# ZGC-SP/mpcith_kyber_kosk

Measured on AMD Instinct MI355X. Metric: kyber768_kosk_proofs_per_sec_prove_plus_verify, higher is better.
Workload: dtype u16

## Files before the change

mpcith_kyber_kosk_amd/csrc/kosk_ctx.cpp:

```cpp
#include "kosk_ctx.hpp"

#include <atomic>

#include <chrono>
#include <cstdio>
#include <cstring>
#include <ctime>
#include <thread>

#include "kosk_math.hpp"

namespace kosk {

#define HIPCHK(x) KOSK_HIPCHK(x)

static double now_sec()
{
    return std::chrono::duration<double>(std::chrono::steady_clock::now().time_since_epoch()).count();
}

template <typename T>
static hipError_t dalloc(T **p, size_t n)
{
    return hipMalloc(reinterpret_cast<void **>(p), n * sizeof(T));
// ... 32 lines not shown
        if (pool) pool_destroy(pool);
        if (ev) (void)hipEventDestroy(ev);
        if (ev_kg) (void)hipEventDestroy(ev_kg);
        for (auto e : timer_ev)
            if (e) (void)hipEventDestroy(e);
        return;
    }
    void *dev[] = {t_expand.dfrag, t_recon_d.dfrag, t_recon_2d.dfrag, d_fresh_rows, d_gemm1_rows, d_gemm2_rows, d_off, d_fields, d_asm_groups, d_asm_elems,
                   d_rowtab, d_P, d_tape, d_seedbuf, d_dig1, d_dig2, d_proof, d_A, d_se, d_kg, d_sehat, d_t, d_alpha, d_I, d_pwT, d_coef, d_lin_rows,
                   d_gather, d_gather2, d_O, d_w, d_ell, d_sec, d_sec_u1, d_sec_u2, d_fail, d_inv, d_invlimb, d_vfields,
                   d_vrowtab, d_rows_bg, d_rows_isrc, d_rows_idst, d_rows_u, d_fact, d_invfact, d_node_of, d_isort, d_hrange, d_odig};
    for (void *p : dev)
        if (p) (void)hipFree(p);
    void *host[] = {h_err, h_tape, h_seedbuf, h_dig, h_dig2, h_proof, h_alpha, h_I, h_fail, h_Iimg, h_kg, h_odig};
    for (void *p : host)
        if (p) (void)hipHostFree(p);
    if (d_compact) (void)hipFree(d_compact);
    if (d_compact_bad) (void)hipFree(d_compact_bad);
    if (h_compact) (void)hipHostFree(h_compact);
    if (h_compact_bad) (void)hipHostFree(h_compact_bad);
    if (pool) pool_destroy(pool);
    if (ev) (void)hipEventDestroy(ev);
    if (ev_kg) (void)hipEventDestroy(ev_kg);
    for (auto e : timer_ev)
        if (e) (void)hipEventDestroy(e);
    if (stream) (void)hipStreamDestroy(stream);
}

static int upload_table(Ctx &c, GemmTable &t, const std::vector<uint16_t> &A, int M, int Kdim)
{
    t.M = M;
    t.Mpad = (M + 127) / 128 * 128;
    t.KS = (Kdim + 63) / 64;
    std::vector<uint8_t> pk;
    pack_frag_table(A, M, Kdim, t.Mpad, t.KS, pk);
    HIPCHK(dalloc(&t.dfrag, pk.size()));
    HIPCHK(hipMemcpyAsync(t.dfrag, pk.data(), pk.size(), hipMemcpyHostToDevice, c.stream));
    HIPCHK(hipStreamSynchronize(c.stream));
    return 0;
}

static hipError_t commit_hash_batch(Ctx &c, const HashArgs &ha, int n, int K, bool view, hipStream_t st)
{
    c.prof_begin(view ? PR_HASH_VIEW : PR_HASH_TCOMM, n);
    int variant = 0;
    const hipError_t e = launch_commit_hash(ha, n, K, view, st, &variant);
    if (!c.capturing) c.path_n[(variant & 1) ? PATH_HASH_DMA : PATH_HASH_PLAIN]++;
    c.prof_end(view ? PR_HASH_VIEW : PR_HASH_TCOMM);
    return e;
}

int device_error_check(Ctx &c)
{
    if (!c.h_err) return 0;
    const uint32_t e = *reinterpret_cast<volatile uint32_t *>(c.h_err);
    if (!e) return 0;
    *reinterpret_cast<volatile uint32_t *>(c.h_err) = 0;
    c.err = (e & DEVERR_XOF_BLOCKS) ? "gen_matrix: SHAKE128 block limit reached before 256 coefficients were accepted (indcpa.c:124-145 would squeeze on; "
                                      "probability < 2^-300 with the default limit of 32 blocks): no result was produced"
                                    : "a kernel reported an internal error";
    return -1;
}

hipError_t copy_round_table(Ctx &c, uint8_t *h_dst, const uint8_t *d_src, int n)
{
    return hipMemcpyAsync(h_dst, d_src, (size_t)n * NPARTY * 32, hipMemcpyDeviceToHost, c.stream);
}

// ... 39 lines not shown
        const double keep = est * 0.3 > 100.0 ? est * 0.3 : 100.0;
        double nap_us = est - keep;
        if (nap_us > 200000.0) nap_us = 200000.0;
        struct timespec ts;
        ts.tv_sec = 0;
        ts.tv_nsec = (long)(nap_us * 1e3);
        nanosleep(&ts, nullptr);
        const hipError_t q = hipEventQuery(ev);
        if (q == hipSuccess) overslept = true;
        else if (q != hipErrorNotReady) return q;
    }
    const hipError_t e = overslept ? hipSuccess : hipEventSynchronize(ev);
    const double took = (now_sec() - t0) * 1e6;
    if (overslept) {
        for (int i = 0; i < Ctx::WAIT_HIST; i++) h->us[i] = 0;
        h->at = 0;
    } else {
        h->us[h->at] = took > 1.0 ? took : 1.0;
        h->at = (h->at + 1) % Ctx::WAIT_HIST;
    }
    return e;
}
hipError_t stream_sync_site(Ctx &c, int site, int n)
{
    if (c.blocking_sync || !c.wait_nap) return stream_sync(c);
    const hipError_t e = hipEventRecord(c.ev_sync, c.stream);
    return e != hipSuccess ? e : wait_event(c, c.ev_sync, site, n);
}

int gemm_modq(Ctx &c, const GemmTable &t, const GemmSrc &s, const GemmDst &d, int npg, int ngroups)
{
    if (npg <= 0 || ngroups <= 0) return 0;
    GemmArgs ga{};
    ga.Afrag = t.dfrag; ga.Mpad = t.Mpad; ga.M = t.M; ga.KS = t.KS;
    ga.src = s.src; ga.src_gstride = s.gstride; ga.src_rows = s.rows; ga.src_rstride = s.rstride; ga.src_koff = s.koff;
    ga.src_canonical = s.canonical;
    ga.C = d.C; ga.c_gstride = d.gstride; ga.c_rows = d.rows; ga.c_rstride = d.rstride; ga.c_off = d.off;
    ga.npg = npg; ga.ngroups = ngroups;
    if (!table_gemm_ok(ga)) { c.err = "internal: table_gemm_ok() refuses the operands of a mod-q product"; return -1; }
    HIPCHK(launch_table_gemm(ga, c.stream));
    if (!c.capturing) c.path_n[PATH_TABLE_GEMM]++;
    return 0;
}

template <typename T>
static int upload_vec(Ctx &c, T **d, const std::vector<T> &v)
{
    HIPCHK(dalloc(d, v.size() ? v.size() : 1));
    if (!v.empty()) {
        HIPCHK(hipMemcpyAsync(*d, v.data(), v.size() * sizeof(T), hipMemcpyHostToDevice, c.stream));
        HIPCHK(hipStreamSynchronize(c.stream));
    }
    return 0;
}

static int build_tables(Ctx &c)
{
    const Params &P = c.P;
    const RowMap &rm = c.rm;
    const int K = P.K, M = P.M, E = P.E, Z = P.Z;

    {
        std::vector<uint16_t> A((size_t)EXP_M * XLEN, 0);
        for (int m = 0; m < EXP_M; m++) {
            const int x = EXP_OFF + m;
            if (x < XLEN) A[(size_t)m * XLEN + x] = 1;
            else if (x < NPTS) lagrange_row(&A[(size_t)m * XLEN], XLEN, 0, x);
// ... 790 lines not shown
```

mpcith_kyber_kosk_amd/csrc/kosk_ctx.hpp:

```cpp
#pragma once
#include <hip/hip_runtime.h>

#include <string>
#include <functional>
#include <vector>

#include "kosk_device.hpp"
#include "kosk_host.hpp"
#include "kosk_params.hpp"

#define KOSK_HIPCHK(x)                                                      \
    do {                                                                    \
        hipError_t e_ = (x);                                                \
        if (e_ != hipSuccess) {                                             \
            (void)hipGetLastError();                                        \
            c.err = std::string(#x) + ": " + hipGetErrorString(e_);         \
            return -1;                                                      \
        }                                                                   \
    } while (0)

namespace kosk {

typedef void (*randombytes_fn)(void *user, uint8_t *out, size_t len);
typedef void (*round_fn)(void *user, int role, int round, const void *d_digests, size_t bytes);
// ... 2 lines not shown
    const uint8_t *tapes;
    size_t tape_stride;
    uint8_t *pk, *sk;
    int count = 0;
    const KeygenIn *next = nullptr;
    round_fn hook = nullptr;
    void *hook_user = nullptr;
    const uint8_t *seeds = nullptr;
    size_t seed_stride = 0;
};
struct VerifySeg {
    int count;
    const uint8_t *pk;
    uint8_t *ok;
    const VerifySeg *next = nullptr;
    round_fn hook = nullptr;
    void *hook_user = nullptr;
};

enum Phase { PH_HOST_PRE = 0, PH_GPU_COMMIT, PH_FS_ALPHA, PH_GPU_RELATION, PH_FS_OPEN, PH_GPU_ASSEMBLE, PH_D2H,
             PH_P1_ISSUE, PH_P2_ISSUE, PH_P3_ISSUE, PH_V1_ISSUE, PH_V1_WAIT, PH_V_FS_ALPHA, PH_V2_ISSUE, PH_V2_WAIT, PH_V_FS_OPEN,
             PH_COUNT };

enum ProfId { PR_HASH_TCOMM = 0, PR_HASH_VIEW, PR_GEMM_EXPAND1, PR_GEMM_EXPAND2, PR_LINCOMB, PR_NTT_F, PR_ASSEMBLE,
              PR_V_HASH_TCOMM, PR_V_HASH_VIEW, PR_V_INTERP_BUILD, PR_V_GEMM_INTERP, PR_V_GEMM_EXPAND, PR_V_GEMM_RECON,
              PR_V_LINCOMB, PR_FS_ALPHA, PR_FS_OPENED, PR_V_FS_ALPHA, PR_V_FS_OPENED, PR_COUNT };

enum PathId { PATH_HASH_DMA = 0, PATH_HASH_PLAIN, PATH_TABLE_GEMM, PATH_LIMB_GEMM, PATH_COPY_DIRECT, PATH_COPY_STAGED,
              PATH_GRAPH_REPLAY, PATH_DIGEST_COPY, PATH_SMALL_COPY_KERNEL, PATH_FS_DEVICE, PATH_FS_HOST, PATH_TAPE_EXPAND, PATH_COUNT };

struct GemmTable {
    uint8_t *dfrag = nullptr;
    int M = 0, Mpad = 0, KS = 0;
};

struct GemmSrc {
    const uint16_t *src;
    size_t gstride;
    const int16_t *rows;
    int rstride, koff;
    int canonical = 1;
};
struct GemmDst {
    uint16_t *C;
    size_t gstride;
    const int16_t *rows;
    int rstride, off;
};

struct CompactField {
    uint32_t src_off, dst_off, n;
    int raw;
};
struct CompactPlan {
    CompactField f[NFIELDS];
    size_t bytes;
};
CompactPlan make_compact_plan(const Params &P);
int compact_encode(const Params &P, const uint8_t *img, uint8_t *out);
void compact_decode(const Params &P, const uint8_t *in, uint8_t *img);

struct Ctx {
    int device = 0;
    Params P{};
    RowMap rm{};
    int max_batch = 0;
// ... 234 lines not shown
```

mpcith_kyber_kosk_amd/csrc/kosk_device.hpp:

```cpp
#pragma once
#include <hip/hip_runtime.h>

#include "kosk_params.hpp"

namespace kosk {

struct XofGuard {
    uint32_t *err = nullptr;
    int max_blocks = 32;
};
enum : uint32_t { DEVERR_XOF_BLOCKS = 1u };


struct HashArgs {
    const uint16_t *rows;
    size_t group_stride;
    int row_stride;
    int col_off;
    int lanes_per_group;
    const uint8_t *prefix;
    uint8_t *out;
    int out_lanes_per_group;
};

struct NttArgs {
    const int16_t *in;
    const int32_t *src_off;
    size_t in_gstride;
    int16_t *out;
    const int32_t *dst_off;
    size_t out_gstride;
    int npg;
    int npoly;
    int out_canonical;
    uint32_t *cmp_fail;
    int cmp_delta, cmp_bit;
    uint32_t npg_magic;
};
inline uint32_t ntt_npg_magic(int npg) { return npg <= 1 ? 0xFFFFFFFFu : (uint32_t)((1ull << 32) / (uint32_t)npg); }

KOSK_HD inline int limb_swz(int r) { return (-(r >> 2)) & 3; }
KOSK_HD inline size_t limb_offset(int r, int k, int limb, int RT)
{
    const int ks = k >> 6, kc = (k >> 4) & 3, rr = r & 15;
    return ((size_t)(ks * RT + (r >> 4)) * 2 + limb) * 1024 + rr * 64 + ((kc ^ limb_swz(rr)) << 4) + (k & 15);
}
KOSK_HD inline void limb_split(int32_t centred, int &c0, int &c1)
{
    c0 = ((centred + 32) & 63) - 32;
    c1 = (centred - c0) >> 6;
}

struct GemmArgs {
    const uint8_t *Afrag;
    int Mpad, M, KS;
    const uint16_t *src;
    size_t src_gstride;
    const int16_t *src_rows;
    int src_rstride, src_koff;
    uint16_t *C;
    size_t c_gstride;
    const int16_t *c_rows;
    int c_rstride;
    int c_off;
    int npg;
    int src_canonical;
    int ngroups;
};

struct LincombArgs {
    uint16_t *P;
    size_t proof_stride;
    uint16_t *O;
    size_t o_stride;
    RowMap rm;
    int J;
    const int32_t *pwT;
    int ncols;
    const uint16_t *col_map;
    int col_map_stride;
    int nxb, njc, ngroups;
};

struct FieldDesc {
    uint32_t off;
    int sel;
    int width;
    int rowtab_off;
// ... 193 lines not shown
```

mpcith_kyber_kosk_amd/csrc/kosk_host.cpp:

```cpp
#include "kosk_host.hpp"

#include <linux/futex.h>
#include <sched.h>
#include <sys/random.h>
#include <sys/syscall.h>
#include <unistd.h>

#include <algorithm>
#include <atomic>
#include <chrono>
#include <mutex>
#include <stdexcept>
#include <cstdio>
#include <cstdlib>
#include <cstring>
#include <vector>
#include <thread>

#include "kosk_math.hpp"

namespace kosk {

namespace {

// ... 494 lines not shown
                e >>= 1;
            }
            inv[a] = (uint16_t)r;
        }
    }
};
const InvTable &inv_table()
{
    static const InvTable t;
    return t;
}
}

uint16_t gf_inv_host(uint16_t a) { return inv_table().inv[a % Q]; }

void lagrange_row(uint16_t *row, int n, int a, int t)
{
    std::vector<uint32_t> pre(n + 1), suf(n + 1), fact(n + 1);
    fact[0] = 1;
    for (int i = 1; i <= n; i++) fact[i] = fact[i - 1] * (uint32_t)i % Q;
    auto diff = [&](int m) { return (uint32_t)((((t - a - m) % Q) + Q) % Q); };
    pre[0] = 1;
    for (int m = 0; m < n; m++) pre[m + 1] = pre[m] * diff(m) % Q;
    suf[n] = 1;
    for (int m = n - 1; m >= 0; m--) suf[m] = suf[m + 1] * diff(m) % Q;
    for (int j = 0; j < n; j++) {
        const uint32_t num = pre[j] * suf[j + 1] % Q;
        uint32_t den = fact[j] * fact[n - 1 - j] % Q;
        if ((n - 1 - j) & 1) den = (Q - den) % Q;
        row[j] = (uint16_t)(num * gf_inv_host((uint16_t)den) % Q);
    }
}

void pack_frag_table(const std::vector<uint16_t> &A, int M, int Kdim, int Mpad, int KS, std::vector<uint8_t> &out)
{
    const int RT = Mpad / 16;
    out.assign((size_t)KS * RT * 2048, 0);
    for (int m = 0; m < M; m++)
        for (int k = 0; k < Kdim; k++) {
            const int32_t c = gf_center(A[(size_t)m * Kdim + k]);
            const int c0 = ((c + 32) & 63) - 32, c1 = (c - c0) >> 6;
            const int ks = k >> 6, kc = (k >> 4) & 3, rr = m & 15;
            const size_t base = ((size_t)(ks * RT + (m >> 4)) * 2) * 1024 + (size_t)(kc * 16 + rr) * 16 + (k & 15);
            out[base] = (uint8_t)(int8_t)c0;
            out[base + 1024] = (uint8_t)(int8_t)c1;
        }
}

class Pool {
public:
    static Pool &get() { static Pool p; return p; }
    Pool() = default;
    ~Pool()
    {
        stop_.store(true);
        gen_.fetch_add(1);
        wake(INT32_MAX);
        for (auto &t : th_) t.join();
    }
    void run(int n, int nthreads, const std::function<void(int)> &fn)
    {
        std::lock_guard<std::mutex> job_lock(job_mu_);
        grow(nthreads - 1);
        Job job{&fn, n, std::min<int>((int)th_.size(), nthreads - 1)};
        cur_.store(&job);
        gen_.fetch_add(1);
        if (sleepers_.load() > 0) wake(job.want);
        work(job);
        while (job.done.load(std::memory_order_acquire) < n) __builtin_ia32_pause();
        cur_.store(nullptr);
        while (inside_.load() != 0) __builtin_ia32_pause();
        if (job.failed.load()) throw std::runtime_error("exception in a host worker job");
    }

private:
// ... 135 lines not shown
```

mpcith_kyber_kosk_amd/csrc/kosk_host.hpp:

```cpp
#pragma once
#include <cstddef>
#include <cstdint>
#include <functional>
#include <vector>

#include "kosk_params.hpp"

namespace kosk {

void sha3_256(uint8_t out[32], const uint8_t *in, size_t inlen);
void sha3_512(uint8_t out[64], const uint8_t *in, size_t inlen);
void shake128(uint8_t *out, size_t outlen, const uint8_t *in, size_t inlen);
void shake256(uint8_t *out, size_t outlen, const uint8_t *in, size_t inlen);
void shake256_prf(uint8_t *out, size_t outlen, const uint8_t key[32], uint8_t nonce);

struct HostKey {
    int16_t A[MAXK * MAXK * 256];
    int16_t se[2 * MAXK * 256];
    int16_t t[MAXK * 256];
};
void host_keygen(const Params &P, const uint8_t seed64[64], uint8_t *pk, uint8_t *sk, HostKey &key);
void host_decode_pk(const Params &P, const uint8_t *pk, HostKey &key);

void fs_alpha(const Params &P, const uint8_t *tcomm_all , uint16_t *alpha );
void fs_opened(const uint8_t *digests_all , uint16_t I[NOPEN], uint16_t rest[NREST]);

void lagrange_row(uint16_t *row, int n, int a, int t);
uint16_t gf_inv_host(uint16_t a);

void pack_frag_table(const std::vector<uint16_t> &A, int M, int Kdim, int Mpad, int KS, std::vector<uint8_t> &out);

class Pool;
Pool *pool_create();
void pool_destroy(Pool *);
int pool_reserve(Pool *, int nthreads);
int host_cpu_count();
void parallel_for(Pool *pool, int n, int nthreads, const std::function<void(int)> &fn);
inline void parallel_for(int n, int nthreads, const std::function<void(int)> &fn) { parallel_for(nullptr, n, nthreads, fn); }

void sha3_256_multi(uint8_t *out, const uint8_t *const *in, size_t len, int count);
int sha3_multi_width();

void assemble_digest_table(uint8_t *table, const uint16_t *I, const uint8_t *unopened, const uint8_t *opened);

void fs_alpha_batch(const Params &P, int n, const uint8_t *digs, size_t dig_stride, uint16_t *alpha, size_t alpha_stride, int nthreads, Pool *pool = nullptr,
                    const std::function<void(int)> *prep = nullptr);
void fs_opened_batch(int n, const uint8_t *digs, size_t dig_stride, uint16_t *I, uint16_t *rest, size_t sel_stride, int nthreads, Pool *pool = nullptr,
                     bool windows = false, const std::function<void(int)> *prep = nullptr);

void os_randombytes(uint8_t *out, size_t len);

constexpr int SEED_BYTES = 32;
void tape_from_seed(const Params &P, const uint8_t seed[SEED_BYTES], uint8_t *tape);

}
```

mpcith_kyber_kosk_amd/csrc/kosk_kernels.hip:

```cpp
#include <hip/hip_runtime.h>

#include <cstdlib>
#include <utility>

#include "kosk_device.hpp"
#include "kosk_keccak_dev.hpp"
#include "kosk_keccak_split_dev.hpp"
#include "kosk_keygen_dev.hpp"
#include "kosk_keygen_wave_dev.hpp"
#include "kosk_math.hpp"
#include "kosk_limb_dev.hpp"

namespace kosk {

template <int PREFIX_WORDS, int NROWS, bool PIPE>
__global__ __launch_bounds__(64) void k_commit_hash(HashArgs a)
{
    const int lane = blockIdx.x * 64 + threadIdx.x;
    const int g = blockIdx.y;
    if (lane >= a.lanes_per_group) return;
    const uint16_t *__restrict__ base = a.rows + (size_t)g * a.group_stride + a.col_off + lane;
    const size_t dig = ((size_t)g * a.out_lanes_per_group + lane) * 32;

    constexpr int W = PREFIX_WORDS + NROWS;
// ... 675 lines not shown
__global__ __launch_bounds__(128) void k_matvec_ntt(const int16_t *__restrict__ A, size_t A_stride,
                                                    uint16_t *__restrict__ P, size_t proof_stride, int v_row0, int row0, int K)
{
    matvec_ntt_item(A, A_stride, P, proof_stride, v_row0, row0, K, threadIdx.x, blockIdx.x, blockIdx.y);
}

__global__ __launch_bounds__(256) void k_relation_ntt(NttArgs na, const int16_t *__restrict__ A, size_t A_stride, uint16_t *P,
                                                      size_t proof_stride, RowMap rm)
{
    __shared__ __attribute__((aligned(16))) int16_t lds[NTT_PPB * NTT_LSTRIDE];
    const int b = blockIdx.x, K = rm.K, tid = threadIdx.x;
    NttArgs a = na;
    a.in += (size_t)b * na.in_gstride;
    a.out += (size_t)b * na.out_gstride;
    a.npoly = a.npg;
    ntt256_tile(a, 0, lds);
    __syncthreads();
    for (int idx = tid; idx < K * 128; idx += 256) matvec_ntt_item(A, A_stride, P, proof_stride, rm.nttsr, rm.nttasr, K, idx & 127, idx >> 7, b);
    if (tid <= NOPEN) {
        uint16_t *Pb = P + (size_t)b * proof_stride + NSEC + tid;
        for (int i = 0; i < K; i++) {
            const uint16_t sv = Pb[(size_t)(rm.sr + i) * RS], ev = Pb[(size_t)(rm.er + i) * RS];
            Pb[(size_t)(rm.nttsr + i) * RS] = sv;
            Pb[(size_t)(rm.nttasr + i) * RS] = sv;
            Pb[(size_t)(rm.ntter + i) * RS] = ev;
        }
    }
}


constexpr int TG_WAVES = 8;

template <int KS, int TG_RT, int NBT>
__global__ __launch_bounds__(512, (KS <= 7 && NBT == 3) ? 2 : 1) void k_table_gemm(GemmArgs a, int nchunks, int chunks_per_block, int nblk, int msplit, int wide_stores)
{
    constexpr int TG_CHUNK = 16 * TG_RT, TG_NB = 16 * NBT;
    __shared__ __attribute__((aligned(16))) uint8_t ldsB[KS * NBT * 2048];
    const int tid = threadIdx.x, lane = tid & 63, w = tid >> 6;
    const int ntot = a.npg * a.ngroups;
    const int vid = xcd_virtual_id();
    const int bxr = vid / msplit, byr = vid - bxr * msplit;
    if (bxr >= nblk) return;
    const int n0 = bxr * TG_NB;

    constexpr int ITEMS = TG_NB * KS * 4, PER = (ITEMS + 511) / 512;
    uint4 x0[PER], x1[PER];
#pragma unroll
    for (int q = 0; q < PER; q++) {
        const int item = tid + q * 512;
        const int row_l = item / (KS * 4), kc16 = item - row_l * (KS * 4);
        const int n = n0 + row_l;
        x0[q] = make_uint4(0, 0, 0, 0);
        x1[q] = x0[q];
        if (item < ITEMS && n < ntot) {
            const int g = n / a.npg, i = n - g * a.npg;
            const uint16_t *src = a.src + (size_t)g * a.src_gstride + (size_t)(a.src_rows ? (int)a.src_rows[i] : i) * a.src_rstride + a.src_koff + kc16 * 16;
            x0[q] = *reinterpret_cast<const uint4 *>(src);
            x1[q] = *reinterpret_cast<const uint4 *>(src + 8);
        }
    }
#pragma unroll
    for (int q = 0; q < PER; q++) {
        const int item = tid + q * 512;
        if (item < ITEMS) {
            const int row_l = item / (KS * 4), kc16 = item - row_l * (KS * 4);
            uint4 lo, hi;
            gm_split16(x0[q], x1[q], lo, hi);
// ... 68 lines not shown
#pragma unroll
        for (int ks = 0; ks < KS; ks++) {
            v4i(&bc)[2 * NBT] = ks == 0 ? fb0 : fb[ks & 1];
            v4i(&bn)[2 * NBT] = ks + 1 == KS ? fb0 : fb[(ks & 1) ^ 1];
            load_b(ks + 1 < KS ? ks + 1 : 0, bn);
            __builtin_amdgcn_sched_barrier(0);
#pragma unroll
            for (int i = 0; i < TG_RT; i++) {
#pragma unroll
                for (int j = 0; j < NBT; j++) s0[i][j] = __builtin_amdgcn_mfma_i32_16x16x64_i8(fa[ks][2 * i], bc[2 * j], ks == 0 ? zero4 : s0[i][j], 0, 0, 0);
#pragma unroll
                for (int j = 0; j < NBT; j++) s1[i][j] = __builtin_amdgcn_mfma_i32_16x16x64_i8(fa[ks][2 * i], bc[2 * j + 1], ks == 0 ? zero4 : s1[i][j], 0, 0, 0);
#pragma unroll
                for (int j = 0; j < NBT; j++) s1[i][j] = __builtin_amdgcn_mfma_i32_16x16x64_i8(fa[ks][2 * i + 1], bc[2 * j], s1[i][j], 0, 0, 0);
#pragma unroll
                for (int j = 0; j < NBT; j++) s2[i][j] = __builtin_amdgcn_mfma_i32_16x16x64_i8(fa[ks][2 * i + 1], bc[2 * j + 1], ks == 0 ? zero4 : s2[i][j], 0, 0, 0);
            }
            load_chunk_ks(cn, ks, fa[ks]);
            __builtin_amdgcn_sched_barrier(0);
        }
        uint2 pk[NBT];
#pragma unroll
        for (int j = 0; j < NBT; j++) {
            uint32_t v[4];
#pragma unroll
            for (int r = 0; r < 4; r++) v[r] = gf_reduce_limbs(s0[0][j][r], s1[0][j][r], s2[0][j][r]);
            pk[j] = make_uint2(v[0] | (v[1] << 16), v[2] | (v[3] << 16));
            if (j & 1) store_pair(j - 1, c, pk[j - 1], pk[j]);
            else if (j == NBT - 1) store_one(j, c, pk[j]);
        }
    }
}

template <int KS, int NBT, bool CANON>
__global__ __launch_bounds__(512, 1) void k_table_gemm_p(GemmArgs a, int nchunks, int nblk, int wide_stores, uint32_t npg_magic)
{
    auto split = [&](int n, int &g, int &i) {
        uint32_t gg = __umulhi((uint32_t)n, npg_magic);
        int r = n - (int)gg * a.npg;
        if (r >= a.npg) { gg++; r -= a.npg; }
        g = (int)gg;
        i = r;
    };
    constexpr int TG_RT = 1, TG_CHUNK = 16, TG_NB = 16 * NBT, BUF = KS * NBT * 2048;
    __shared__ __attribute__((aligned(16))) uint8_t ldsB[2 * BUF];
    const int tid = threadIdx.x, lane = tid & 63, w = tid >> 6;
    const int ntot = a.npg * a.ngroups;
    const long total = (long)nblk * nchunks;
    const long u0 = (long)blockIdx.x * total / gridDim.x, u1 = (long)(blockIdx.x + 1) * total / gridDim.x;
    if (u0 >= u1) return;
    int rb = (int)(u0 / nchunks), ca = (int)(u0 - (long)rb * nchunks);
    long u = u0;

    constexpr int ITEMS = TG_NB * KS * 4, PER = (ITEMS + 511) / 512;
    auto item_src = [&](int blk, int item) -> const uint16_t * {
        const int row_l = item / (KS * 4), kc16 = item - row_l * (KS * 4);
        const int n = blk * TG_NB + row_l;
        if (item >= ITEMS || n >= ntot) return nullptr;
        int g, i;
        split(n, g, i);
        return a.src + (size_t)g * a.src_gstride + (size_t)(a.src_rows ? (int)a.src_rows[i] : i) * a.src_rstride + a.src_koff + kc16 * 16;
    };
    auto item_put = [&](int buf, int item, const uint4 &x0, const uint4 &x1) {
        if (item >= ITEMS) return;
        const int row_l = item / (KS * 4), kc16 = item - row_l * (KS * 4);
        uint4 lo, hi;
        if constexpr (CANON) gm_split16_pk(x0, x1, lo, hi);
        else gm_split16(x0, x1, lo, hi);
        uint8_t *d = ldsB + buf * BUF + ((kc16 >> 2) * NBT + (row_l >> 4)) * 2048 + (row_l & 15) * 64 + (((kc16 & 3) ^ limb_swz(row_l & 15)) << 4);
        *reinterpret_cast<uint4 *>(d) = lo;
        *reinterpret_cast<uint4 *>(d + 1024) = hi;
    };
    {
        uint4 x0[PER], x1[PER];
#pragma unroll
        for (int q = 0; q < PER; q++) {
            const uint16_t *src = item_src(rb, tid + q * 512);
            x0[q] = make_uint4(0, 0, 0, 0);
            x1[q] = x0[q];
            if (src) { x0[q] = *reinterpret_cast<const uint4 *>(src); x1[q] = *reinterpret_cast<const uint4 *>(src + 8); }
        }
#pragma unroll
        for (int q = 0; q < PER; q++) item_put(0, tid + q * 512, x0[q], x1[q]);
    }
    const int ART = a.Mpad / 16;
    const int frag = (lane & 15) * 64 + (((lane >> 4) ^ limb_swz(lane & 15)) << 4);
    v4i fa[KS][2 * TG_RT];
    auto load_chunk_ks = [&](int c, int ks, v4i (&dst)[2 * TG_RT]) {
        const uint8_t *src = a.Afrag + ((size_t)(ks * ART + TG_RT * c) * 2) * 1024 + lane * 16;
#pragma unroll
        for (int q = 0; q < 2 * TG_RT; q++) dst[q] = *reinterpret_cast<const v4i *>(src + q * 1024);
    };
    {
        const int c_first = ca + w < nchunks ? ca + w : 0;
#pragma unroll
        for (int ks = 0; ks < KS; ks++) load_chunk_ks(c_first, ks, fa[ks]);
    }
    __syncthreads();
    const v4i zero4 = {0, 0, 0, 0}, bias4 = {LIMB_BIAS, LIMB_BIAS, LIMB_BIAS, LIMB_BIAS};
    const int grp = lane >> 4;
    int buf = 0;
    while (u < u1) {
        const int cb = (long)(nchunks - ca) <= u1 - u ? nchunks : ca + (int)(u1 - u);
        const bool have_next = u + (cb - ca) < u1;
        const uint8_t *lds_cur = ldsB + buf * BUF;
        uint16_t *crow[NBT];
#pragma unroll
        for (int j = 0; j < NBT; j++) {
            const int n = rb * TG_NB + j * 16 + (lane & 15);
            crow[j] = nullptr;
            if (n < ntot) {
                int g, i;
                split(n, g, i);
                crow[j] = a.C + (size_t)g * a.c_gstride + (size_t)(a.c_rows ? (int)a.c_rows[i] : i) * a.c_rstride + a.c_off + (lane >> 4) * 4;
            }
        }
        auto store_pair = [&](int j, int c, uint2 pj, uint2 pk) {
            if (wide_stores) {
                const auto sx = __builtin_amdgcn_permlane16_swap(pj.x, pk.x, false, false);
                const auto sy = __builtin_amdgcn_permlane16_swap(pj.y, pk.y, false, false);
                uint16_t *p = (grp & 1) ? (crow[j + 1] ? crow[j + 1] - 4 : nullptr) : crow[j];
                if (p) *reinterpret_cast<uint4 *>(p + c * TG_CHUNK) = make_uint4(sx[0], sy[0], sx[1], sy[1]);
            } else {
                if (crow[j]) *reinterpret_cast<uint2 *>(crow[j] + c * TG_CHUNK) = pj;
                if (crow[j + 1]) *reinterpret_cast<uint2 *>(crow[j + 1] + c * TG_CHUNK) = pk;
            }
        };
        auto store_one = [&](int j, int c, uint2 pj) {
            if (crow[j]) *reinterpret_cast<uint2 *>(crow[j] + c * TG_CHUNK) = pj;
        };
        v4i fb[2][2 * NBT], fb0[2 * NBT];
        auto load_b = [&](int ks, v4i (&dst)[2 * NBT]) {
            const uint8_t *lb = lds_cur + ks * NBT * 2048 + frag;
#pragma unroll
            for (int j = 0; j < NBT; j++) {
                dst[2 * j] = *reinterpret_cast<const v4i *>(lb + j * 2048);
                dst[2 * j + 1] = *reinterpret_cast<const v4i *>(lb + j * 2048 + 1024);
            }
        };
        int it = 0;
        const int c_first = ca + w;
        const int nmy = c_first < cb ? (cb - c_first + TG_WAVES - 1) / TG_WAVES : 0;
        if (nmy > 0) load_b(0, fb0);
        for (int ci = 0; ci < nmy; ci++) {
            const int c = c_first + ci * TG_WAVES;
            const int cn = ci + 1 < nmy ? c + TG_WAVES : (have_next && w < nchunks ? w : c);
            uint4 nx0 = make_uint4(0, 0, 0, 0), nx1 = nx0;
            const bool fetch = have_next && it < PER;
            if (fetch) {
                const uint16_t *src = item_src(rb + 1, tid + it * 512);
                if (src) { nx0 = *reinterpret_cast<const uint4 *>(src); nx1 = *reinterpret_cast<const uint4 *>(src + 8); }
            }
            v4i s0[NBT], s1[NBT], s2[NBT];
#pragma unroll
            for (int ks = 0; ks < KS; ks++) {
                v4i(&bc)[2 * NBT] = ks == 0 ? fb0 : fb[ks & 1];
                v4i(&bn)[2 * NBT] = ks + 1 == KS ? fb0 : fb[(ks & 1) ^ 1];
                load_b(ks + 1 < KS ? ks + 1 : 0, bn);
                __builtin_amdgcn_sched_barrier(0);
#pragma unroll
                for (int j = 0; j < NBT; j++) s0[j] = __builtin_amdgcn_mfma_i32_16x16x64_i8(fa[ks][0], bc[2 * j], ks == 0 ? bias4 : s0[j], 0, 0, 0);
#pragma unroll
                for (int j = 0; j < NBT; j++) s1[j] = __builtin_amdgcn_mfma_i32_16x16x64_i8(fa[ks][0], bc[2 * j + 1], ks == 0 ? zero4 : s1[j], 0, 0, 0);
#pragma unroll
                for (int j = 0; j < NBT; j++) s1[j] = __builtin_amdgcn_mfma_i32_16x16x64_i8(fa[ks][1], bc[2 * j], s1[j], 0, 0, 0);
#pragma unroll
                for (int j = 0; j < NBT; j++) s2[j] = __builtin_amdgcn_mfma_i32_16x16x64_i8(fa[ks][1], bc[2 * j + 1], ks == 0 ? zero4 : s2[j], 0, 0, 0);
                load_chunk_ks(cn, ks, fa[ks]);
                __builtin_amdgcn_sched_barrier(0);
            }
            uint2 pk[NBT];
#pragma unroll
            for (int j = 0; j < NBT; j++) {
                uint32_t v[4];
#pragma unroll
                for (int r = 0; r < 4; r++) v[r] = gf_reduce_limbs_biased_lazy(s0[j][r], s1[j][r], s2[j][r]);
                pk[j] = make_uint2(gf_canon_pair(v[0], v[1]), gf_canon_pair(v[2], v[3]));
                if (j & 1) store_pair(j - 1, c, pk[j - 1], pk[j]);
                else if (j == NBT - 1) store_one(j, c, pk[j]);
            }
            if (fetch) { item_put(buf ^ 1, tid + it * 512, nx0, nx1); it++; }
        }
        if (have_next) {
            for (; it < PER; it++) {
                const uint16_t *src = item_src(rb + 1, tid + it * 512);
                uint4 nx0 = make_uint4(0, 0, 0, 0), nx1 = nx0;
                if (src) { nx0 = *reinterpret_cast<const uint4 *>(src); nx1 = *reinterpret_cast<const uint4 *>(src + 8); }
                item_put(buf ^ 1, tid + it * 512, nx0, nx1);
            }
            if (nmy == 0 && w < nchunks) {
#pragma unroll
                for (int ks = 0; ks < KS; ks++) load_chunk_ks(w, ks, fa[ks]);
            }
        }
        u += cb - ca;
        rb++;
        ca = 0;
        buf ^= 1;
        lds_barrier();
    }
}

constexpr int LC_JPAD = 80;
constexpr int LF_A_BYTES = 2 * 8 * 2048, LF_B_BYTES = 2 * 8 * 2048;

constexpr int LS_JT = 5;
constexpr int LS_A_BYTES = 2 * 8 * 2048;
constexpr int LS_B_BYTES = 2 * LS_JT * 2048;
__global__ __launch_bounds__(256, 2) void k_lincomb_stream(const uint16_t *P, size_t proof_stride, int row_f, int row_tf, int M,
                                                           const uint8_t *__restrict__ coef, int BRT, uint16_t *C,
                                                           const int16_t *__restrict__ lin_rows, int J, int K, int row_s, int row_e,
                                                           int row_sr, int row_er, int ngroups)
{
    __shared__ __attribute__((aligned(16))) uint8_t lds[LS_A_BYTES + LS_B_BYTES];
    uint8_t *ldsB = lds + LS_A_BYTES;
    const int tid = threadIdx.x, lane = tid & 63, w = tid >> 6;
    constexpr int MB = (NPTS + 127) / 128;
    const int total = ngroups * MB;
    const int fb0 = (int)(((long)blockIdx.x * total) / gridDim.x), fb1 = (int)(((long)(blockIdx.x + 1) * total) / gridDim.x);
    if (fb0 >= fb1) return;
    const int pp = tid & 63, c4 = tid >> 6, xl = pp * 2;
    uint32_t raw[20];
    auto gload = [&](int fb) {
        const int g = fb / MB, m0 = (fb - g * MB) * 128;
        const uint16_t *src = P + (size_t)(g >> 1) * proof_stride + (size_t)((g & 1) ? row_tf : row_f) * RS + (m0 + xl < NPTS ? m0 + xl : 0);
// ... 602 lines not shown
{
    if (args.npoly <= 0) return hipSuccess;
    NttArgs a = args;
    a.npg_magic = ntt_npg_magic(a.npg);
    const bool plain = !a.src_off && !a.dst_off && !a.cmp_fail && (a.npg >= a.npoly || (a.in_gstride == (size_t)a.npg * 256 && a.out_gstride == (size_t)a.npg * 256)) &&
                       (reinterpret_cast<uintptr_t>(a.in) & 15) == 0 && (reinterpret_cast<uintptr_t>(a.out) & 15) == 0;
    const dim3 grid((a.npoly + NTT_PPB - 1) / NTT_PPB);
    if (plain) hipLaunchKernelGGL(k_ntt256<true>, grid, dim3(256), 0, st, a);
    else hipLaunchKernelGGL(k_ntt256<false>, grid, dim3(256), 0, st, a);
    return hipGetLastError();
}

hipError_t launch_relation_ntt(const NttArgs &na, const int16_t *A, size_t A_stride, uint16_t *P, size_t proof_stride, const RowMap &rm,
                               int nproofs, hipStream_t st)
{
    if (na.npg > NTT_PPB) return hipErrorInvalidValue;
    NttArgs nb = na;
    nb.npg_magic = ntt_npg_magic(nb.npg);
    hipLaunchKernelGGL(k_relation_ntt, dim3(nproofs), dim3(256), 0, st, nb, A, A_stride, P, proof_stride, rm);
    return hipGetLastError();
}

hipError_t launch_matvec_ntt(const int16_t *A, size_t A_stride, uint16_t *P, size_t proof_stride, int v_row0, int row0, int K,
                             int nproofs, hipStream_t st)
{
    hipLaunchKernelGGL(k_matvec_ntt, dim3(K, nproofs), dim3(128), 0, st, A, A_stride, P, proof_stride, v_row0, row0, K);
    return hipGetLastError();
}

static_assert(RS % 8 == 0 && NSEC % 8 == 0 && EXP_OFF % 4 == 0 && EXP_M % 32 == 0 && NSEC % 32 == 0,
              "row stride, source offsets, output offsets and table heights of the library's own products");
bool table_gemm_ok(const GemmArgs &a)
{
    return a.Afrag && (a.KS == 7 || a.KS == 13) && a.M % 32 == 0 && a.src_koff % 8 == 0 && a.src_rstride % 8 == 0 &&
           a.src_gstride % 8 == 0 && (reinterpret_cast<uintptr_t>(a.src) & 15) == 0 && a.c_off % 4 == 0 && a.c_rstride % 4 == 0 &&
           a.c_gstride % 4 == 0 && (reinterpret_cast<uintptr_t>(a.C) & 7) == 0;
}

hipError_t launch_table_gemm(const GemmArgs &a, hipStream_t st)
{
    const int ntot = a.npg * a.ngroups;
    if (ntot <= 0) return hipSuccess;
    static const int ncu = [] {
        int dev = 0, cus = 256;
        if (hipGetDevice(&dev) != hipSuccess || hipDeviceGetAttribute(&cus, hipDeviceAttributeMultiprocessorCount, dev) != hipSuccess || cus <= 0) { (void)hipGetLastError(); cus = 256; }
        return cus;
    }();
    const int nblk = (ntot + 47) / 48, nchunks = a.M / 16;
    const int ws = a.c_off % 8 == 0 && a.c_rstride % 8 == 0 && a.c_gstride % 8 == 0 && (reinterpret_cast<uintptr_t>(a.C) & 15) == 0;
    if (a.KS == 7) {
        const long total = (long)nblk * nchunks;
        long nwg = total / 8 < ncu ? total / 8 : ncu;
        if (nwg < 1) nwg = 1;
        const uint32_t magic = ntt_npg_magic(a.npg);
        if (a.src_canonical) hipLaunchKernelGGL((k_table_gemm_p<7, 3, true>), dim3((unsigned)nwg), dim3(512), 0, st, a, nchunks, nblk, ws, magic);
        else hipLaunchKernelGGL((k_table_gemm_p<7, 3, false>), dim3((unsigned)nwg), dim3(512), 0, st, a, nchunks, nblk, ws, magic);
        return hipGetLastError();
    }
    int msplit = nblk >= 160 ? 1 : (256 + nblk - 1) / nblk;
    if (msplit > nchunks) msplit = nchunks;
    const int cpb = (nchunks + msplit - 1) / msplit;
    msplit = (nchunks + cpb - 1) / cpb;
    const dim3 grid((unsigned)((nblk * msplit + 7) / 8 * 8));
    hipLaunchKernelGGL((k_table_gemm<13, 1, 3>), grid, dim3(512), 0, st, a, nchunks, cpb, nblk, msplit, ws);
    return hipGetLastError();
}

// ... 68 lines not shown
```

Measured before the change: 184,300.

## Use 32-deep MFMA tail step for KS=7 table GEMM, packing half-size tail

Result: slower. 171,500 (-6.9%).

```diff
diff --git a/mpcith_kyber_kosk_amd/csrc/kosk_ctx.cpp b/mpcith_kyber_kosk_amd/csrc/kosk_ctx.cpp
--- a/mpcith_kyber_kosk_amd/csrc/kosk_ctx.cpp
+++ b/mpcith_kyber_kosk_amd/csrc/kosk_ctx.cpp
@@ -88,8 +88,9 @@
     t.M = M;
     t.Mpad = (M + 127) / 128 * 128;
     t.KS = (Kdim + 63) / 64;
+    t.tail32 = Kdim - (t.KS - 1) * 64 <= 32;
     std::vector<uint8_t> pk;
-    pack_frag_table(A, M, Kdim, t.Mpad, t.KS, pk);
+    pack_frag_table(A, M, Kdim, t.Mpad, t.KS, t.tail32 != 0, pk);
     HIPCHK(dalloc(&t.dfrag, pk.size()));
     HIPCHK(hipMemcpyAsync(t.dfrag, pk.data(), pk.size(), hipMemcpyHostToDevice, c.stream));
     HIPCHK(hipStreamSynchronize(c.stream));
@@ -195,7 +196,7 @@
 {
     if (npg <= 0 || ngroups <= 0) return 0;
     GemmArgs ga{};
-    ga.Afrag = t.dfrag; ga.Mpad = t.Mpad; ga.M = t.M; ga.KS = t.KS;
+    ga.Afrag = t.dfrag; ga.Mpad = t.Mpad; ga.M = t.M; ga.KS = t.KS; ga.tail32 = t.tail32;
     ga.src = s.src; ga.src_gstride = s.gstride; ga.src_rows = s.rows; ga.src_rstride = s.rstride; ga.src_koff = s.koff;
     ga.src_canonical = s.canonical;
     ga.C = d.C; ga.c_gstride = d.gstride; ga.c_rows = d.rows; ga.c_rstride = d.rstride; ga.c_off = d.off;
diff --git a/mpcith_kyber_kosk_amd/csrc/kosk_ctx.hpp b/mpcith_kyber_kosk_amd/csrc/kosk_ctx.hpp
--- a/mpcith_kyber_kosk_amd/csrc/kosk_ctx.hpp
+++ b/mpcith_kyber_kosk_amd/csrc/kosk_ctx.hpp
@@ -58,6 +58,7 @@
 struct GemmTable {
     uint8_t *dfrag = nullptr;
     int M = 0, Mpad = 0, KS = 0;
+    int tail32 = 0;
 };
 
 struct GemmSrc {
diff --git a/mpcith_kyber_kosk_amd/csrc/kosk_device.hpp b/mpcith_kyber_kosk_amd/csrc/kosk_device.hpp
--- a/mpcith_kyber_kosk_amd/csrc/kosk_device.hpp
+++ b/mpcith_kyber_kosk_amd/csrc/kosk_device.hpp
@@ -54,6 +54,7 @@
 struct GemmArgs {
     const uint8_t *Afrag;
     int Mpad, M, KS;
+    int tail32;
     const uint16_t *src;
     size_t src_gstride;
     const int16_t *src_rows;
diff --git a/mpcith_kyber_kosk_amd/csrc/kosk_host.cpp b/mpcith_kyber_kosk_amd/csrc/kosk_host.cpp
--- a/mpcith_kyber_kosk_amd/csrc/kosk_host.cpp
+++ b/mpcith_kyber_kosk_amd/csrc/kosk_host.cpp
@@ -550,15 +550,22 @@
     }
 }
 
-void pack_frag_table(const std::vector<uint16_t> &A, int M, int Kdim, int Mpad, int KS, std::vector<uint8_t> &out)
+void pack_frag_table(const std::vector<uint16_t> &A, int M, int Kdim, int Mpad, int KS, bool tail32, std::vector<uint8_t> &out)
 {
     const int RT = Mpad / 16;
-    out.assign((size_t)KS * RT * 2048, 0);
+    const size_t tail_base = (size_t)(KS - 1) * RT * 2048;
+    out.assign(tail32 ? tail_base + (size_t)RT * 1024 : (size_t)KS * RT * 2048, 0);
     for (int m = 0; m < M; m++)
         for (int k = 0; k < Kdim; k++) {
             const int32_t c = gf_center(A[(size_t)m * Kdim + k]);
             const int c0 = ((c + 32) & 63) - 32, c1 = (c - c0) >> 6;
             const int ks = k >> 6, kc = (k >> 4) & 3, rr = m & 15;
+            if (tail32 && ks == KS - 1) {
+                const size_t base = tail_base + ((size_t)(m >> 4) * 2) * 512 + (size_t)(((k >> 3) & 3) * 16 + rr) * 8 + (k & 7);
+                out[base] = (uint8_t)(int8_t)c0;
+                out[base + 512] = (uint8_t)(int8_t)c1;
+                continue;
+            }
             const size_t base = ((size_t)(ks * RT + (m >> 4)) * 2) * 1024 + (size_t)(kc * 16 + rr) * 16 + (k & 15);
             out[base] = (uint8_t)(int8_t)c0;
             out[base + 1024] = (uint8_t)(int8_t)c1;
diff --git a/mpcith_kyber_kosk_amd/csrc/kosk_host.hpp b/mpcith_kyber_kosk_amd/csrc/kosk_host.hpp
--- a/mpcith_kyber_kosk_amd/csrc/kosk_host.hpp
+++ b/mpcith_kyber_kosk_amd/csrc/kosk_host.hpp
@@ -28,7 +28,7 @@
 void lagrange_row(uint16_t *row, int n, int a, int t);
 uint16_t gf_inv_host(uint16_t a);
 
-void pack_frag_table(const std::vector<uint16_t> &A, int M, int Kdim, int Mpad, int KS, std::vector<uint8_t> &out);
+void pack_frag_table(const std::vector<uint16_t> &A, int M, int Kdim, int Mpad, int KS, bool tail32, std::vector<uint8_t> &out);
 
 class Pool;
 Pool *pool_create();
diff --git a/mpcith_kyber_kosk_amd/csrc/kosk_kernels.hip b/mpcith_kyber_kosk_amd/csrc/kosk_kernels.hip
--- a/mpcith_kyber_kosk_amd/csrc/kosk_kernels.hip
+++ b/mpcith_kyber_kosk_amd/csrc/kosk_kernels.hip
@@ -731,7 +731,7 @@
 constexpr int TG_WAVES = 8;
 
 template <int KS, int TG_RT, int NBT>
-__global__ __launch_bounds__(512, (KS <= 7 && NBT == 3) ? 2 : 1) void k_table_gemm(GemmArgs a, int nchunks, int chunks_per_block, int nblk, int msplit, int wide_stores)
+__global__ __launch_bounds__(512, 1) void k_table_gemm(GemmArgs a, int nchunks, int chunks_per_block, int nblk, int msplit, int wide_stores)
 {
     constexpr int TG_CHUNK = 16 * TG_RT, TG_NB = 16 * NBT;
     __shared__ __attribute__((aligned(16))) uint8_t ldsB[KS * NBT * 2048];
@@ -866,9 +866,11 @@
     }
 }
 
+static_assert(XLEN <= 6 * 64 + 32, "k_table_gemm_p: six 64-deep k-steps and one 32-deep");
 template <int KS, int NBT, bool CANON>
 __global__ __launch_bounds__(512, 1) void k_table_gemm_p(GemmArgs a, int nchunks, int nblk, int wide_stores, uint32_t npg_magic)
 {
+    static_assert(KS == 7, "six full k-steps and the 32-deep one (GemmArgs::tail32)");
     auto split = [&](int n, int &g, int &i) {
         uint32_t gg = __umulhi((uint32_t)n, npg_magic);
         int r = n - (int)gg * a.npg;
@@ -876,7 +878,12 @@
         g = (int)gg;
         i = r;
     };
-    constexpr int TG_RT = 1, TG_CHUNK = 16, TG_NB = 16 * NBT, BUF = KS * NBT * 2048;
+    constexpr int KF = KS - 1;
+    constexpr int KC = KF * 4 + 2;
+    constexpr int TG_CHUNK = 16, TG_NB = 16 * NBT;
+    constexpr int TAIL = KF * NBT * 2048;
+    constexpr int BUF = TAIL + NBT * 1024;
+    static_assert(2 * BUF <= 160 * 1024, "LDS budget of one CU");
     __shared__ __attribute__((aligned(16))) uint8_t ldsB[2 * BUF];
     const int tid = threadIdx.x, lane = tid & 63, w = tid >> 6;
     const int ntot = a.npg * a.ngroups;
@@ -886,9 +893,9 @@
     int rb = (int)(u0 / nchunks), ca = (int)(u0 - (long)rb * nchunks);
     long u = u0;
 
-    constexpr int ITEMS = TG_NB * KS * 4, PER = (ITEMS + 511) / 512;
+    constexpr int ITEMS = TG_NB * KC, PER = (ITEMS + 511) / 512;
     auto item_src = [&](int blk, int item) -> const uint16_t * {
-        const int row_l = item / (KS * 4), kc16 = item - row_l * (KS * 4);
+        const int row_l = item / KC, kc16 = item - row_l * KC;
         const int n = blk * TG_NB + row_l;
         if (item >= ITEMS || n >= ntot) return nullptr;
         int g, i;
@@ -897,13 +904,20 @@
     };
     auto item_put = [&](int buf, int item, const uint4 &x0, const uint4 &x1) {
         if (item >= ITEMS) return;
-        const int row_l = item / (KS * 4), kc16 = item - row_l * (KS * 4);
+        const int row_l = item / KC, kc16 = item - row_l * KC, r = row_l & 15;
         uint4 lo, hi;
         if constexpr (CANON) gm_split16_pk(x0, x1, lo, hi);
         else gm_split16(x0, x1, lo, hi);
-        uint8_t *d = ldsB + buf * BUF + ((kc16 >> 2) * NBT + (row_l >> 4)) * 2048 + (row_l & 15) * 64 + (((kc16 & 3) ^ limb_swz(row_l & 15)) << 4);
-        *reinterpret_cast<uint4 *>(d) = lo;
-        *reinterpret_cast<uint4 *>(d + 1024) = hi;
+        if (kc16 < KF * 4) {
+            uint8_t *d = ldsB + buf * BUF + ((kc16 >> 2) * NBT + (row_l >> 4)) * 2048 + r * 64 + (((kc16 & 3) ^ limb_swz(r)) << 4);
+            *reinterpret_cast<uint4 *>(d) = lo;
+            *reinterpret_cast<uint4 *>(d + 1024) = hi;
+        } else {
+            uint8_t *d = ldsB + buf * BUF + TAIL + (row_l >> 4) * 1024 + r * 64;
+            const int ch = (kc16 - KF * 4) * 2;
+            *reinterpret_cast<uint4 *>(d + ((ch ^ limb_swz(r)) << 4)) = make_uint4(lo.x, lo.y, hi.x, hi.y);
+            *reinterpret_cast<uint4 *>(d + (((ch + 1) ^ limb_swz(r)) << 4)) = make_uint4(lo.z, lo.w, hi.z, hi.w);
+        }
     };
     {
         uint4 x0[PER], x1[PER];
@@ -919,19 +933,28 @@
     }
     const int ART = a.Mpad / 16;
     const int frag = (lane & 15) * 64 + (((lane >> 4) ^ limb_swz(lane & 15)) << 4);
-    v4i fa[KS][2 * TG_RT];
-    auto load_chunk_ks = [&](int c, int ks, v4i (&dst)[2 * TG_RT]) {
-        const uint8_t *src = a.Afrag + ((size_t)(ks * ART + TG_RT * c) * 2) * 1024 + lane * 16;
-#pragma unroll
-        for (int q = 0; q < 2 * TG_RT; q++) dst[q] = *reinterpret_cast<const v4i *>(src + q * 1024);
+    v4i fa[KF][2];
+    long fat[2];
+    auto load_chunk_ks = [&](int c, int ks, v4i (&dst)[2]) {
+        const uint8_t *src = a.Afrag + ((size_t)(ks * ART + c) * 2) * 1024 + lane * 16;
+        dst[0] = *reinterpret_cast<const v4i *>(src);
+        dst[1] = *reinterpret_cast<const v4i *>(src + 1024);
+    };
+    auto load_chunk_tail = [&](int c) {
+        const uint8_t *src = a.Afrag + (size_t)KF * ART * 2048 + (size_t)c * 1024 + lane * 8;
+        fat[0] = *reinterpret_cast<const long *>(src);
+        fat[1] = *reinterpret_cast<const long *>(src + 512);
     };
     {
         const int c_first = ca + w < nchunks ? ca + w : 0;
 #pragma unroll
-        for (int ks = 0; ks < KS; ks++) load_chunk_ks(c_first, ks, fa[ks]);
+        for (int ks = 0; ks < KF; ks++) load_chunk_ks(c_first, ks, fa[ks]);
+        load_chunk_tail(c_first);
     }
     __syncthreads();
     const v4i zero4 = {0, 0, 0, 0}, bias4 = {LIMB_BIAS, LIMB_BIAS, LIMB_BIAS, LIMB_BIAS};
+    auto lo64 = [](const v4i &v) { return (long)(((unsigned long)(uint32_t)v[1] << 32) | (uint32_t)v[0]); };
+    auto hi64 = [](const v4i &v) { return (long)(((unsigned long)(uint32_t)v[3] << 32) | (uint32_t)v[2]); };
     const int grp = lane >> 4;
     int buf = 0;
     while (u < u1) {
@@ -964,6 +987,12 @@
             if (crow[j]) *reinterpret_cast<uint2 *>(crow[j] + c * TG_CHUNK) = pj;
         };
         v4i fb[2][2 * NBT], fb0[2 * NBT];
+        v4i fbt[NBT];
+        auto load_bt = [&]() {
+            const uint8_t *lb = lds_cur + TAIL + frag;
+#pragma unroll
+            for (int j = 0; j < NBT; j++) fbt[j] = *reinterpret_cast<const v4i *>(lb + j * 1024);
+        };
         auto load_b = [&](int ks, v4i (&dst)[2 * NBT]) {
             const uint8_t *lb = lds_cur + ks * NBT * 2048 + frag;
 #pragma unroll
@@ -987,10 +1016,10 @@
             }
             v4i s0[NBT], s1[NBT], s2[NBT];
 #pragma unroll
-            for (int ks = 0; ks < KS; ks++) {
+            for (int ks = 0; ks < KF; ks++) {
                 v4i(&bc)[2 * NBT] = ks == 0 ? fb0 : fb[ks & 1];
-                v4i(&bn)[2 * NBT] = ks + 1 == KS ? fb0 : fb[(ks & 1) ^ 1];
-                load_b(ks + 1 < KS ? ks + 1 : 0, bn);
+                if (ks + 1 < KF) load_b(ks + 1, fb[(ks & 1) ^ 1]);
+                else load_bt();
                 __builtin_amdgcn_sched_barrier(0);
 #pragma unroll
                 for (int j = 0; j < NBT; j++) s0[j] = __builtin_amdgcn_mfma_i32_16x16x64_i8(fa[ks][0], bc[2 * j], ks == 0 ? bias4 : s0[j], 0, 0, 0);
@@ -1003,6 +1032,20 @@
                 load_chunk_ks(cn, ks, fa[ks]);
                 __builtin_amdgcn_sched_barrier(0);
             }
+            load_b(0, fb0);
+            __builtin_amdgcn_sched_barrier(0);
+#pragma unroll
+            for (int j = 0; j < NBT; j++) s0[j] = __builtin_amdgcn_mfma_i32_16x16x32_i8(fat[0], lo64(fbt[j]), s0[j], 0, 0, 0);
+#pragma unroll
+            for (int j = 0; j < NBT; j++) s1[j] = __builtin_amdgcn_mfma_i32_16x16x32_i8(fat[0], hi64(fbt[j]), s1[j], 0, 0, 0);
+#pragma unroll
+            for (int j = 0; j < NBT; j++) s1[j] = __builtin_amdgcn_mfma_i32_16x16x32_i8(fat[1], lo64(fbt[j]), s1[j], 0, 0, 0);
+#pragma unroll
+            for (int j = 0; j < NBT; j++) s2[j] = __builtin_amdgcn_mfma_i32_16x16x32_i8(fat[1], hi64(fbt[j]), s2[j], 0, 0, 0);
+            load_chunk_tail(cn);
+            __builtin_amdgcn_sched_barrier(0);
+            asm volatile("s_nop 15");
+            __builtin_amdgcn_sched_barrier(0);
             uint2 pk[NBT];
 #pragma unroll
             for (int j = 0; j < NBT; j++) {
@@ -1024,7 +1067,8 @@
             }
             if (nmy == 0 && w < nchunks) {
 #pragma unroll
-                for (int ks = 0; ks < KS; ks++) load_chunk_ks(w, ks, fa[ks]);
+                for (int ks = 0; ks < KF; ks++) load_chunk_ks(w, ks, fa[ks]);
+                load_chunk_tail(w);
             }
         }
         u += cb - ca;
@@ -1693,7 +1737,7 @@
               "row stride, source offsets, output offsets and table heights of the library's own products");
 bool table_gemm_ok(const GemmArgs &a)
 {
-    return a.Afrag && (a.KS == 7 || a.KS == 13) && a.M % 32 == 0 && a.src_koff % 8 == 0 && a.src_rstride % 8 == 0 &&
+    return a.Afrag && ((a.KS == 7 && a.tail32) || (a.KS == 13 && !a.tail32)) && a.M % 32 == 0 && a.src_koff % 8 == 0 && a.src_rstride % 8 == 0 &&
            a.src_gstride % 8 == 0 && (reinterpret_cast<uintptr_t>(a.src) & 15) == 0 && a.c_off % 4 == 0 && a.c_rstride % 4 == 0 &&
            a.c_gstride % 4 == 0 && (reinterpret_cast<uintptr_t>(a.C) & 7) == 0;
 }
```
